# cxzheng/sprsolve

Hardware: AMD Instinct MI355X
Metric: BiCGStab iterations/s (f64, 50M-row 7-point 3-D Poisson) + CSR SpMV GB/s vs HBM roofline (higher is better)
Workload: dtype f64

## Files before the change

### sprsolve_amd/csrc/spmv_chain.hip

```cpp
#include "spmv_dict_dev.hpp"
#include "bicg_fuse.hpp"

namespace sprs {
namespace {

constexpr int CH_ROWS = CH_B * 2 * WAVE;
constexpr int CH_W = TILE_W;
constexpr int CH_WL = CH_ROWS + 2 * CH_W;

struct NoPro { __device__ __forceinline__ bool prologue() { return true; } };
template <int FUSE, class PRO, int DOT, bool UX, int UL, bool TRI, bool YST = true, int UPD = 0>
__global__ __launch_bounds__(BLOCK) void spmv_chain_kernel(const int4 *__restrict__ tiles, const int2 *__restrict__ segs, const int32_t *__restrict__ xstart,
                                                           const BlkDesc *__restrict__ desc, const TilePat pat,
                                                           int n_left, const int32_t *__restrict__ left_order,
                                                           const int32_t *__restrict__ row_ptr, const uint8_t *__restrict__ code,
                                                           const int32_t *__restrict__ off_tab, const double *__restrict__ val_tab,
                                                           const double *__restrict__ x, double *__restrict__ y, const double *__restrict__ u,
                                                           double *__restrict__ part0, double *__restrict__ part1,
                                                           const int *__restrict__ status, int nrows, int ncols, const Fin fin,
                                                           PRO pro, const double *__restrict__ in1, const double *__restrict__ in2,
                                                           double *__restrict__ own) {
    using T = double;
    constexpr int NV = FUSE == 0 ? 1 : FUSE;
    static_assert(FUSE == 0 || (FUSE == 2 && DOT == 2 && UX && UPD == 0) || (FUSE == 3 && DOT == 1 && !UX) ||
                  (FUSE == 2 && DOT == 0 && !UX && !YST && UPD != 0), "fused flavours: K3 into K4, K1 into K2, K5 on the chains");
    static_assert((YST || FUSE == 2) && (UPD == 0 || FUSE == 2), "only BiCGStab's K4 / K5 drop the y store");
    constexpr int W = CH_W, WL = CH_WL;
    constexpr int NW = WL / 2 / BLOCK;
    constexpr int NQ = CH_B / NWAVE;
    constexpr int NN = UL - 2;
    constexpr int TC = NN / 2;
    static_assert(WL % (2 * BLOCK) == 0 && CH_B % NWAVE == 0 && NN >= 1 && UL <= 8 && (!TRI || (NN & 1)), "chain shape");
    static_assert(sizeof(T) * WL >= sizeof(uint32_t) * NWAVE * CW2, "the left walk's code slices live in the first window");
    __shared__ __attribute__((aligned(16))) T win[3][WL];
    __shared__ PairEnt<T> s_pair[TAB];
    __shared__ T red[NWAVE];
    const int run_state = status != nullptr ? *status : (int)ST_RUNNING;
    const int tid = threadIdx.x, lane = tid & (WAVE - 1);
    const int wv = __builtin_amdgcn_readfirstlane(tid >> 6);
    stage_pair(s_pair, tid, off_tab[tid] * 8, val_tab[tid]);
    __syncthreads();
    if (run_state != ST_RUNNING) { fin_idle(fin, DOT == 2); return; }
    [[maybe_unused]] T c0 = 0.0, c1 = 0.0;
    [[maybe_unused]] T nw = 0.0;
    if constexpr (FUSE != 0) {
        if (!pro.prologue()) return;
        if constexpr (FUSE == 2) c0 = pro.na; else { c0 = pro.a; c1 = pro.beta; }
        if constexpr (UPD != 0) nw = pro.nw;
    }
    T d0 = 0.0, d1 = 0.0;

    const int Pf = pat.off[UL - 1];
    const int xhi = (ncols - 2) & ~1;
    const int xcd = blockIdx.x & 7;
    const int sstep = gridDim.x >> 3;
    const int send = xstart[xcd + 1];
    constexpr int PF = (FUSE == 3 || UPD != 0) ? 1 : 2;
    struct WinRegs { u4v a[NW]; u4v b[NV >= 2 ? NW : 1]; u4v c[NV == 3 ? NW : 1]; };
    WinRegs R0;
    [[maybe_unused]] WinRegs R1;
    auto issue = [&](int tw, WinRegs &R) {
#pragma unroll
        for (int i = 0; i < NW; ++i) {
            int g = tw - W + 2 * (tid + i * BLOCK);
            g = g < 0 ? 0 : (g > xhi ? xhi : g);
            R.a[i] = *reinterpret_cast<const u4v *>(x + g);
            if constexpr (NV >= 2) R.b[i] = *reinterpret_cast<const u4v *>(in1 + g);
            if constexpr (NV == 3) R.c[i] = *reinterpret_cast<const u4v *>(in2 + g);
        }
    };
    auto stage = [&](int slot, const WinRegs &R) {
#pragma unroll
        for (int i = 0; i < NW; ++i) {
            if constexpr (FUSE == 0) {
                *reinterpret_cast<u4v *>(&win[slot][2 * (tid + i * BLOCK)]) = R.a[i];
            } else {
                D2 a, b, cc{0.0, 0.0};
                __builtin_memcpy(&a, &R.a[i], 16); __builtin_memcpy(&b, &R.b[i], 16);
                if constexpr (NV == 3) __builtin_memcpy(&cc, &R.c[i], 16);
                const D2 o = FUSE == 2 ? D2{comb_k3(a.lo, b.lo, c0), comb_k3(a.hi, b.hi, c0)}
                                       : D2{comb_k1(a.lo, b.lo, cc.lo, c0, c1), comb_k1(a.hi, b.hi, cc.hi, c0, c1)};
                *reinterpret_cast<D2 *>(&win[slot][2 * (tid + i * BLOCK)]) = o;
            }
        }
    };
    for (int s = xstart[xcd] + (blockIdx.x >> 3); s < send; s += sstep) {
        const int2 sg = segs[s];
        const int t0 = __builtin_amdgcn_readfirstlane(sg.x), L = __builtin_amdgcn_readfirstlane(sg.y);
        int4 ent = tiles[t0];
        uint32_t rbw[NQ]; int nnw[NQ];
#pragma unroll
        for (int q = 0; q < NQ; ++q) { const BlkDesc d = desc[__builtin_amdgcn_readfirstlane(ent.x) + q * NWAVE + wv]; rbw[q] = (uint32_t)d.rb; nnw[q] = d.nn; }
        __syncthreads();
        int ts_prev = __builtin_amdgcn_readfirstlane(ent.y) - Pf;
        int sp = 0, sc = 1, sn = 2;
        issue(ts_prev, R0); stage(sp, R0);
        issue(__builtin_amdgcn_readfirstlane(ent.y), R0); stage(sc, R0);
        issue(__builtin_amdgcn_readfirstlane(ent.z), R0);
        if constexpr (PF == 2) { if (L > 1) issue(tiles[t0 + 1].z, R1); }
        auto body = [&](int k, WinRegs &RS) {
            const int ts = __builtin_amdgcn_readfirstlane(ent.y), ts_next = __builtin_amdgcn_readfirstlane(ent.z);
            uint32_t rbc[NQ]; int nnc[NQ];
#pragma unroll
            for (int q = 0; q < NQ; ++q) { rbc[q] = rbw[q]; nnc[q] = nnw[q]; }
            stage(sn, RS);
            __syncthreads();
            if (k + PF < L) issue(tiles[t0 + k + PF].z, RS);
            if (k + 1 < L) {
                ent = tiles[t0 + k + 1];
                const int b1 = __builtin_amdgcn_readfirstlane(ent.x);
#pragma unroll
                for (int q = 0; q < NQ; ++q) { const BlkDesc d = desc[b1 + q * NWAVE + wv]; rbw[q] = (uint32_t)d.rb; nnw[q] = d.nn; }
            }
            const int dlo = ts - Pf - ts_prev, dhi = ts + Pf - ts_next;
            const T *wp = &win[sp][W + dlo], *wc = &win[sc][W], *wn = &win[sn][W + dhi];
            D2 uu[NQ];
            if (DOT != 0 && !UX) {
#pragma unroll
                for (int q = 0; q < NQ; ++q) {
                    const u4v w4 = __builtin_nontemporal_load(reinterpret_cast<const u4v *>(u + (ts + ((q * NWAVE + wv) << 7) + 2 * lane)));
                    __builtin_memcpy(&uu[q], &w4, 16);
                }
            }
            struct UpdRegs { u4v x, p, q, t; };
            [[maybe_unused]] UpdRegs ur[2];
            [[maybe_unused]] auto upd_load = [&](int q, UpdRegs &U) {
                if constexpr (UPD != 0) {
                    const int g = ts + ((q * NWAVE + wv) << 7) + 2 * lane;
                    U.x = __builtin_nontemporal_load(reinterpret_cast<const u4v *>(pro.x + g));
                    U.p = __builtin_nontemporal_load(reinterpret_cast<const u4v *>(pro.y + g));
                    U.q = __builtin_nontemporal_load(reinterpret_cast<const u4v *>(pro.r0 + g));
                    if constexpr (UPD == 2) U.t = __builtin_nontemporal_load(reinterpret_cast<const u4v *>(pro.t + g));
                }
            };
            upd_load(0, ur[0]);
            T opl[UL], oph[UL], ux0 = 0.0, ux1 = 0.0;
            auto read_ops = [&](int q) {
                const int l = ((q * NWAVE + wv) << 7) + 2 * lane;
                const D2 f0 = *reinterpret_cast<const D2 *>(wp + l), f1 = *reinterpret_cast<const D2 *>(wn + l);
                opl[0] = f0.lo; oph[0] = f0.hi; opl[UL - 1] = f1.lo; oph[UL - 1] = f1.hi;
                if constexpr (TRI) {
#pragma unroll
                    for (int t = 0; t < NN; ++t) {
                        if (t == TC - 1 || t == TC + 1) continue;
                        const D2 v2 = *reinterpret_cast<const D2 *>(wc + l + pat.off[1 + t]);
                        opl[1 + t] = v2.lo; oph[1 + t] = v2.hi;
                    }
                    if constexpr (NN >= 3) {
                        const int oc = pat.off[1 + TC];
                        opl[TC] = wc[l + oc - 1]; oph[TC] = opl[1 + TC];
                        opl[2 + TC] = oph[1 + TC]; oph[2 + TC] = wc[l + oc + 2];
                    }
                } else {
#pragma unroll
                    for (int t = 0; t < NN; ++t) { opl[1 + t] = wc[l + pat.off[1 + t]]; oph[1 + t] = wc[l + pat.off[1 + t] + 1]; }
                }
                if ((DOT != 0 && UX) || FUSE != 0) { const D2 c2 = *reinterpret_cast<const D2 *>(wc + l); ux0 = c2.lo; ux1 = c2.hi; }
            };
            read_ops(0);
#pragma unroll
            for (int q = 0; q < NQ; ++q) {
                const uint32_t rbq = (uint32_t)__builtin_amdgcn_readfirstlane((int)rbc[q]);
                T pl[UL], ph[UL];
#pragma unroll
                for (int t = 0; t < UL; ++t) { pl[t] = opl[t]; ph[t] = oph[t]; }
                const T u0 = (DOT != 0 && !UX) ? uu[q].lo : ux0, u1 = (DOT != 0 && !UX) ? uu[q].hi : ux1;
                [[maybe_unused]] const D2 mine{ux0, ux1};
                if (q + 1 < NQ) { read_ops(q + 1); upd_load(q + 1, ur[(q + 1) & 1]); }
                T acc0 = 0.0, acc1 = 0.0;
                if constexpr (UPD == 2) {
                    D2 tt;
                    __builtin_memcpy(&tt, &ur[q & 1].t, 16);
                    acc0 = tt.lo; acc1 = tt.hi;
                } else {
                    pair_fold<UL>(pl, ph, pat.val, rbq, nnc[q], s_pair, lane, acc0, acc1);
                }
                row_pair_out<DOT, YST>(y + (ts + ((q * NWAVE + wv) << 7) + 2 * lane), acc0, acc1, u0, u1, d0, d1);
                if constexpr (UPD != 0) {
                    D2 xx, pp, qq, rr;
                    __builtin_memcpy(&xx, &ur[q & 1].x, 16); __builtin_memcpy(&pp, &ur[q & 1].p, 16); __builtin_memcpy(&qq, &ur[q & 1].q, 16);
                    bicg_k5_row(xx.lo, pp.lo, mine.lo, acc0, qq.lo, c0, nw, rr.lo, d0, d1);
                    bicg_k5_row(xx.hi, pp.hi, mine.hi, acc1, qq.hi, c0, nw, rr.hi, d0, d1);
                    const int g = ts + ((q * NWAVE + wv) << 7) + 2 * lane;
                    u4v xo, ro;
                    __builtin_memcpy(&xo, &xx, 16); __builtin_memcpy(&ro, &rr, 16);
                    __builtin_nontemporal_store(xo, reinterpret_cast<u4v *>(pro.x + g));
                    __builtin_nontemporal_store(ro, reinterpret_cast<u4v *>(own + g));
                }
                if constexpr (FUSE == 3) {
                    u4v ov;
                    __builtin_memcpy(&ov, &mine, 16);
                    __builtin_nontemporal_store(ov, reinterpret_cast<u4v *>(own + (ts + ((q * NWAVE + wv) << 7) + 2 * lane)));
                }
            }
            __syncthreads();
            ts_prev = ts;
            const int o = sp; sp = sc; sc = sn; sn = o;
        };
        if constexpr (PF == 2) {
            for (int k = 0; k < L; k += 2) { body(k, R0); if (k + 1 < L) body(k + 1, R1); }
        } else {
            for (int k = 0; k < L; ++k) body(k, R0);
        }
    }
    if (n_left > 0) {
        __syncthreads();
        uint32_t (*s_c)[CW2] = reinterpret_cast<uint32_t (*)[CW2]>(&win[0][0]);
        for (int i = lane; i < CW2; i += WAVE) s_c[wv][i] = 0;
        if constexpr (FUSE == 0)
            pair2_walk<DOT, true>(n_left, 0, desc, left_order, row_ptr, code, XPlain{reinterpret_cast<const char *>(x)}, y, u, nrows, ncols, s_pair, s_c, d0, d1);
        else if constexpr (UPD != 0)
            pair2_walk<0, true, XFused<2>, false, BicgUpd<UPD>>(n_left, 0, desc, left_order, row_ptr, code,
                                                                XFused<2>{reinterpret_cast<const char *>(x), reinterpret_cast<const char *>(in1), nullptr, c0, c1},
                                                                nullptr, nullptr, nrows, ncols, s_pair, s_c, d0, d1, nullptr,
                                                                BicgUpd<UPD>{pro.x, pro.y, pro.r0, pro.t, own, c0, nw});
        else if constexpr (!YST)
            pair2_walk<DOT, true, XFused<NV>, false>(n_left, 0, desc, left_order, row_ptr, code,
                                                     XFused<NV>{reinterpret_cast<const char *>(x), reinterpret_cast<const char *>(in1), reinterpret_cast<const char *>(in2), c0, c1},
                                                     nullptr, UX ? nullptr : u, nrows, ncols, s_pair, s_c, d0, d1, own);
        else
            pair2_walk<DOT, true, XFused<NV>>(n_left, 0, desc, left_order, row_ptr, code,
                                              XFused<NV>{reinterpret_cast<const char *>(x), reinterpret_cast<const char *>(in1), reinterpret_cast<const char *>(in2), c0, c1},
                                              y, UX ? nullptr : u, nrows, ncols, s_pair, s_c, d0, d1, own);
    }
    spmv_dot_epilogue<DOT>(d0, d1, red, part0, part1, fin);
    if constexpr (UPD != 0) {
        pro.accN = d0; pro.accR = d1;
        pro.epilogue();
    }
}

}

int chain_rows() { return CH_ROWS; }

template <class Kern, class PRO>
int launch_chain(const sprs_csr *A, const SpmvRoute &rt, Kern kern, const double *x, double *y, const double *u, double *part0, double *part1,
                 const int *status, const Fin &fin, const PRO &pro, const double *in1, const double *in2, double *own) {
    sprs_ctx *c = A->ctx;
    const sprs_dict *D = A->dict;
    const sprs_chain_plan &CP = *rt.chain;
    const TilePat tp = tile_pat(CP);
#define SPRS_CSHAPE(U, TR)                                                                                                                 \
    if (CP.ul == U && (CP.tri != 0) == TR)                                                                                                 \
        SPRS_LAUNCH_SPMV(c, kern(std::integral_constant<int, U>{}, std::bool_constant<TR>{}), rt.grid, reinterpret_cast<const int4 *>(CP.tiles), \
                         reinterpret_cast<const int2 *>(CP.segs), CP.xstart, rt.desc, tp, CP.n_left, CP.left, A->row_ptr, D->pair_code, D->pair_off, \
                         reinterpret_cast<const double *>(D->pair_val), x, y, u, part0, part1, status, (int)A->nrows, (int)A->ncols, fin, pro, in1, in2, own);
    SPRS_CHAIN_SHAPES(SPRS_CSHAPE)
#undef SPRS_CSHAPE
    SPRS_HIP_TRY(c, hipGetLastError());
    return SPRS_OK;
}

int launch_chain_pair(const sprs_csr *A, const SpmvRoute &r, const double *x, double *y, int dot_mode, const double *u,
                      double *part0, double *part1, const int *status, const Fin &fin) {
    int rc = SPRS_OK;
    with_dot(dot_mode, u == x, [&](auto dm, auto ux) {
        constexpr int DM = decltype(dm)::value;
        constexpr bool UXV = DM != 0 && decltype(ux)::value;
        rc = launch_chain(A, r, [](auto ul, auto tri) { return &spmv_chain_kernel<0, NoPro, DM, UXV, decltype(ul)::value, decltype(tri)::value>; },
                          x, y, u, part0, part1, status, fin, NoPro{}, nullptr, nullptr, nullptr);
    });
    return rc;
}

int launch_chain_k4f(const sprs_csr *A, const SpmvRoute &rt, const BicgK3<double, double, false> &pro, const double *r, const double *v, double *s_out,
                     double *t, double *partTT, double *partTR, const int *status, bool store_t) {
    typedef BicgK3<double, double, false> K3;
    auto go = [&](auto yst) {
        return launch_chain(A, rt, [](auto ul, auto tri) { return &spmv_chain_kernel<2, K3, 2, true, decltype(ul)::value, decltype(tri)::value, decltype(yst)::value>; },
                            r, t, nullptr, partTT, partTR, status, Fin{}, pro, v, nullptr, s_out);
    };
    return store_t ? go(std::true_type{}) : go(std::false_type{});
}

int launch_chain_k5(const sprs_csr *A, const SpmvRoute &rt, const BicgK5<double, false, true> &pro, double *r_out, bool recompute) {
    typedef BicgK5<double, false, true> K5;
    auto go = [&](auto upd) {
        return launch_chain(A, rt, [](auto ul, auto tri) { return &spmv_chain_kernel<2, K5, 0, false, decltype(ul)::value, decltype(tri)::value, false, decltype(upd)::value>; },
                            pro.r, nullptr, nullptr, nullptr, nullptr, &pro.S->status, Fin{}, pro, pro.sv, nullptr, r_out);
    };
    return recompute ? go(std::integral_constant<int, 1>{}) : go(std::integral_constant<int, 2>{});
}

int launch_chain_k2f(const sprs_csr *A, const SpmvRoute &rt, const BicgK1<double, double, false> &pro, const double *v_old, const double *p, const double *r,
                     double *p_out, double *v_out, const double *r0, double *partB, const int *status) {
    typedef BicgK1<double, double, false> K1;
    return launch_chain(A, rt, [](auto ul, auto tri) { return &spmv_chain_kernel<3, K1, 1, false, decltype(ul)::value, decltype(tri)::value>; },
                        v_old, v_out, r0, partB, nullptr, status, Fin{}, pro, p, r, p_out);
}

}
```

Before: 880.7.

## Prefetch next tile's streamed vectors into a register ring across chain steps

The per-row streaming loads of u and of the BiCGStab update vectors (x, p, r0, t) are moved out of each tile step. Each slot is now reloaded for the next tile right after the current tile consumes it, and the first tile is loaded before the loop, so HBM latency overlaps a whole tile of SpMV work instead of one quarter-step. The non-prefetch PF path splits the last iteration with a compile-time flag so the common steps carry no branch. This costs more live registers (NQ full slots instead of two), which may lower occupancy. On the PF==2 path the final step reloads the current tile's data that is never used.

```diff
diff --git a/sprsolve_amd/csrc/spmv_chain.hip b/sprsolve_amd/csrc/spmv_chain.hip
--- a/sprsolve_amd/csrc/spmv_chain.hip
+++ b/sprsolve_amd/csrc/spmv_chain.hip
@@ -84,6 +84,22 @@
             }
         }
     };
+    constexpr bool RING = UPD != 0 || (DOT != 0 && !UX);
+    struct UpdRegs { u4v x, p, q, t; };
+    [[maybe_unused]] UpdRegs ur[NQ];
+    [[maybe_unused]] D2 uu[NQ];
+    [[maybe_unused]] auto ring_load = [&](int tr, int q) {
+        const int g = tr + ((q * NWAVE + wv) << 7) + 2 * lane;
+        if constexpr (UPD != 0) {
+            ur[q].x = __builtin_nontemporal_load(reinterpret_cast<const u4v *>(pro.x + g));
+            ur[q].p = __builtin_nontemporal_load(reinterpret_cast<const u4v *>(pro.y + g));
+            ur[q].q = __builtin_nontemporal_load(reinterpret_cast<const u4v *>(pro.r0 + g));
+            if constexpr (UPD == 2) ur[q].t = __builtin_nontemporal_load(reinterpret_cast<const u4v *>(pro.t + g));
+        } else {
+            const u4v w4 = __builtin_nontemporal_load(reinterpret_cast<const u4v *>(u + g));
+            __builtin_memcpy(&uu[q], &w4, 16);
+        }
+    };
     for (int s = xstart[xcd] + (blockIdx.x >> 3); s < send; s += sstep) {
         const int2 sg = segs[s];
         const int t0 = __builtin_amdgcn_readfirstlane(sg.x), L = __builtin_amdgcn_readfirstlane(sg.y);
@@ -98,15 +114,19 @@
         issue(__builtin_amdgcn_readfirstlane(ent.y), R0); stage(sc, R0);
         issue(__builtin_amdgcn_readfirstlane(ent.z), R0);
         if constexpr (PF == 2) { if (L > 1) issue(tiles[t0 + 1].z, R1); }
-        auto body = [&](int k, WinRegs &RS) {
+        if constexpr (RING) {
+#pragma unroll
+            for (int q = 0; q < NQ; ++q) ring_load(__builtin_amdgcn_readfirstlane(ent.y), q);
+        }
+        auto body = [&](int k, WinRegs &RS, auto more) {
             const int ts = __builtin_amdgcn_readfirstlane(ent.y), ts_next = __builtin_amdgcn_readfirstlane(ent.z);
             uint32_t rbc[NQ]; int nnc[NQ];
 #pragma unroll
             for (int q = 0; q < NQ; ++q) { rbc[q] = rbw[q]; nnc[q] = nnw[q]; }
             stage(sn, RS);
             __syncthreads();
-            if (k + PF < L) issue(tiles[t0 + k + PF].z, RS);
-            if (k + 1 < L) {
+            if (PF == 1 ? (bool)more : k + PF < L) issue(tiles[t0 + k + PF].z, RS);
+            if (more) {
                 ent = tiles[t0 + k + 1];
                 const int b1 = __builtin_amdgcn_readfirstlane(ent.x);
 #pragma unroll
@@ -114,26 +134,6 @@
             }
             const int dlo = ts - Pf - ts_prev, dhi = ts + Pf - ts_next;
             const T *wp = &win[sp][W + dlo], *wc = &win[sc][W], *wn = &win[sn][W + dhi];
-            D2 uu[NQ];
-            if (DOT != 0 && !UX) {
-#pragma unroll
-                for (int q = 0; q < NQ; ++q) {
-                    const u4v w4 = __builtin_nontemporal_load(reinterpret_cast<const u4v *>(u + (ts + ((q * NWAVE + wv) << 7) + 2 * lane)));
-                    __builtin_memcpy(&uu[q], &w4, 16);
-                }
-            }
-            struct UpdRegs { u4v x, p, q, t; };
-            [[maybe_unused]] UpdRegs ur[2];
-            [[maybe_unused]] auto upd_load = [&](int q, UpdRegs &U) {
-                if constexpr (UPD != 0) {
-                    const int g = ts + ((q * NWAVE + wv) << 7) + 2 * lane;
-                    U.x = __builtin_nontemporal_load(reinterpret_cast<const u4v *>(pro.x + g));
-                    U.p = __builtin_nontemporal_load(reinterpret_cast<const u4v *>(pro.y + g));
-                    U.q = __builtin_nontemporal_load(reinterpret_cast<const u4v *>(pro.r0 + g));
-                    if constexpr (UPD == 2) U.t = __builtin_nontemporal_load(reinterpret_cast<const u4v *>(pro.t + g));
-                }
-            };
-            upd_load(0, ur[0]);
             T opl[UL], oph[UL], ux0 = 0.0, ux1 = 0.0;
             auto read_ops = [&](int q) {
                 const int l = ((q * NWAVE + wv) << 7) + 2 * lane;
@@ -166,11 +166,11 @@
                 for (int t = 0; t < UL; ++t) { pl[t] = opl[t]; ph[t] = oph[t]; }
                 const T u0 = (DOT != 0 && !UX) ? uu[q].lo : ux0, u1 = (DOT != 0 && !UX) ? uu[q].hi : ux1;
                 [[maybe_unused]] const D2 mine{ux0, ux1};
-                if (q + 1 < NQ) { read_ops(q + 1); upd_load(q + 1, ur[(q + 1) & 1]); }
+                if (q + 1 < NQ) read_ops(q + 1);
                 T acc0 = 0.0, acc1 = 0.0;
                 if constexpr (UPD == 2) {
                     D2 tt;
-                    __builtin_memcpy(&tt, &ur[q & 1].t, 16);
+                    __builtin_memcpy(&tt, &ur[q].t, 16);
                     acc0 = tt.lo; acc1 = tt.hi;
                 } else {
                     pair_fold<UL>(pl, ph, pat.val, rbq, nnc[q], s_pair, lane, acc0, acc1);
@@ -178,7 +178,7 @@
                 row_pair_out<DOT, YST>(y + (ts + ((q * NWAVE + wv) << 7) + 2 * lane), acc0, acc1, u0, u1, d0, d1);
                 if constexpr (UPD != 0) {
                     D2 xx, pp, qq, rr;
-                    __builtin_memcpy(&xx, &ur[q & 1].x, 16); __builtin_memcpy(&pp, &ur[q & 1].p, 16); __builtin_memcpy(&qq, &ur[q & 1].q, 16);
+                    __builtin_memcpy(&xx, &ur[q].x, 16); __builtin_memcpy(&pp, &ur[q].p, 16); __builtin_memcpy(&qq, &ur[q].q, 16);
                     bicg_k5_row(xx.lo, pp.lo, mine.lo, acc0, qq.lo, c0, nw, rr.lo, d0, d1);
                     bicg_k5_row(xx.hi, pp.hi, mine.hi, acc1, qq.hi, c0, nw, rr.hi, d0, d1);
                     const int g = ts + ((q * NWAVE + wv) << 7) + 2 * lane;
@@ -192,15 +192,17 @@
                     __builtin_memcpy(&ov, &mine, 16);
                     __builtin_nontemporal_store(ov, reinterpret_cast<u4v *>(own + (ts + ((q * NWAVE + wv) << 7) + 2 * lane)));
                 }
+                if constexpr (RING) { if (PF == 2 || more) ring_load(more ? ts_next : ts, q); }
             }
             __syncthreads();
             ts_prev = ts;
             const int o = sp; sp = sc; sc = sn; sn = o;
         };
         if constexpr (PF == 2) {
-            for (int k = 0; k < L; k += 2) { body(k, R0); if (k + 1 < L) body(k + 1, R1); }
+            for (int k = 0; k < L; k += 2) { body(k, R0, k + 1 < L); if (k + 1 < L) body(k + 1, R1, k + 2 < L); }
         } else {
-            for (int k = 0; k < L; ++k) body(k, R0);
+            for (int k = 0; k + 1 < L; ++k) body(k, R0, std::true_type{});
+            body(L - 1, R0, std::false_type{});
         }
     }
     if (n_left > 0) {
```

Result: no change. 878.8 (-0.2%).
